# Visual-Behavior/aloception-oss

Measured on AMD Instinct MI355X. Metric: frames/sec (whole node) DeformableDETR-R50 inference, higher is better.
Workload: dtype bf16; 1 GPU; DeformableDETR-R50 inference bf16, batch 8 synthetic 1333x800 frames per GPU, random-init weights; launch=hip-graph replay + eager inference(), per_gpu_batch=8, global_batch=8, parallelism=batch-sharded x1, no collective

## Files before the change

### aloception-oss_amd/alo_hip/__init__.py

```python
import ctypes
import warnings
import os
import subprocess

import torch

_PKG_ROOT = os.path.dirname(os.path.dirname(os.path.abspath(__file__)))
LIB_PATH = os.path.join(_PKG_ROOT, "libalo_hotpath.so")
CSRC_DIR = os.path.join(_PKG_ROOT, "csrc")

ALO_F32, ALO_F64, ALO_BF16, ALO_F16 = 0, 1, 2, 3
RESIDENT_AUTO, RESIDENT_ALWAYS = 0, 1
_DTYPE_CODE = {torch.float32: ALO_F32, torch.float64: ALO_F64, torch.bfloat16: ALO_BF16, torch.float16: ALO_F16}


def _half(f16):
    return (torch.bfloat16, torch.float16) if f16 else (torch.bfloat16,)


_lib = None
_warned_inference_tensor = False


def tensor_version(t):
# ... 685 lines not shown
def linear_shortk_supported(x, weight, f16=False):
    return (x.is_cuda and x.dtype in _half(f16) and weight.dtype == x.dtype and x.shape[-1] in (64, 128, 256)
            and weight.dim() == 2 and weight.shape[1] == x.shape[-1] and weight.shape[0] % 64 == 0)


def linear_shortk(x, weight, bias=None, relu=False, residual=None):
    _no_autograd("linear_shortk", x, weight, bias, residual)
    if not linear_shortk_supported(x, weight, f16=True):
        raise RuntimeError("linear_shortk: needs bf16 / fp16 CUDA tensors of one dtype, K in (64, 128, 256) and N % 64 == 0")
    if bias is not None and bias.dtype != x.dtype:
        raise RuntimeError("linear_shortk: bias must have the dtype of x")
    N, K = weight.shape
    x2 = x.reshape(-1, K)
    if not x2.is_contiguous():
        x2 = x2.contiguous()
    y = torch.empty((x2.shape[0], N), dtype=x.dtype, device=x.device)
    M = x2.shape[0]
    if residual is not None:
        residual = residual.reshape(-1, N)
        if residual.shape[0] != M or residual.dtype != x.dtype or not residual.is_contiguous():
            raise RuntimeError("linear_shortk: residual must be a contiguous (M, N) tensor of x's dtype")
    if M:
        nbytes = 2.0 * (x2.numel() + y.numel() * (2 if residual is not None else 1))
        _launch("alo_linear_shortk", x.device, f"linear_shortk/N={N},K={K}", nbytes, 2.0 * M * N * K, x2, weight.contiguous(),
                None if bias is None else bias.contiguous(), residual, y, M, N, K, 1 if relu else 0, _DTYPE_CODE[x.dtype])
    return y.view(*x.shape[:-1], N)


def linear_packed_supported(x, weight, f16=False):
    return (x.is_cuda and x.dtype in _half(f16) and weight.dtype == x.dtype and weight.dim() == 2
            and x.shape[-1] == weight.shape[1] and weight.shape[1] % 256 == 0 and weight.shape[1] >= 512
            and weight.shape[0] % 128 == 0 and not torch.is_grad_enabled())


def linear_packed(x, weight, bias=None, relu=False, residual=None):
    _no_autograd("linear_packed", x, weight, bias, residual)
    if not linear_packed_supported(x, weight, f16=True):
        raise RuntimeError("linear_packed: needs bf16 / fp16 CUDA tensors of one dtype, K % 256 == 0, K >= 512, N % 128 == 0, no autograd")
    x2 = x.reshape(-1, x.shape[-1])
    if not x2.is_contiguous():
        x2 = x2.contiguous()
    M, K = x2.shape
    N = weight.shape[0]
    y = torch.empty((M, N), dtype=x.dtype, device=x.device)
    if residual is not None:
        residual = residual.reshape(M, N)
        if residual.dtype != x.dtype or not residual.is_contiguous():
            raise RuntimeError("linear_packed: residual must be a contiguous (M, N) tensor of the input's dtype")
    if M:
        packed = pack_mfma_b(weight)
        bias_c = None if bias is None else bias.to(x.dtype).contiguous()
        _launch("alo_linear_packed", x.device, f"linear_packed/K={K}/N={N}", 2.0 * (M * K + M * N * (2 if residual is not None else 1)),
                2.0 * M * N * K, x2, packed, bias_c, residual, y, M, N, K, 1 if relu else 0, _DTYPE_CODE[x.dtype])
    return y.view(*x.shape[:-1], N)


def conv1x1_strided_supported(x, weight2d):
    if not (x.dim() == 4 and x.is_cuda and x.is_contiguous(memory_format=torch.channels_last)):
        return False
    if os.environ.get("ALO_CONV1X1_GATHER") == "0":
        return False
    rows = x.permute(0, 2, 3, 1)
    if linear_shortk_supported(rows, weight2d):
        return True
    return linear_packed_supported(rows, weight2d) and (weight2d.shape[0] >= 1024 or tuple(weight2d.shape) == (128, 512))


def conv1x1_strided(x, weight2d, bias, stride, relu=False):
    _no_autograd("conv1x1_strided", x, weight2d, bias)
    if not conv1x1_strided_supported(x, weight2d):
        raise RuntimeError("conv1x1_strided: unsupported dtype / layout / shape")
    n, cin, h, w_ = x.shape
    cout = weight2d.shape[0]
    ho, wo = (h - 1) // stride + 1, (w_ - 1) // stride + 1
    y = torch.empty((n, cout, ho, wo), dtype=x.dtype, device=x.device, memory_format=torch.channels_last)
    packed = not linear_shortk_supported(x.permute(0, 2, 3, 1), weight2d)
    wt = pack_mfma_b(weight2d) if packed else weight2d.contiguous()
    bias_c = None if bias is None else bias.to(x.dtype).contiguous()
    _launch("alo_conv1x1_nhwc", x.device, f"conv1x1_strided/K={cin}/N={cout}", 2.0 * (y.numel() // cout * cin + y.numel()),
            2.0 * y.numel() * cin, x, wt, 1 if packed else 0, bias_c, None, y, n, h, w_, cin, cout, stride, 1 if relu else 0, ALO_BF16)
    return y


def f32_layers_split():
    return os.environ.get("ALO_F32_LAYERS") == "split"


_F32_ROUTED = {
    (64, 64): (0, None),
    (64, 256): (0, None),
    (256, 128): (0, 1 << 18),
    (256, 256): (0, 1 << 14),
    (256, 384): (0, None),
    (256, 512): (0, None),
    (256, 1024): (1 << 14, None),
    (512, 128): (0, None),
}


def _f32_gemm_routed(M, K, N, identity):
    if identity:
        return K <= 512
    lo, hi = _F32_ROUTED.get((K, N), (0, 0))
    return M >= lo and (hi is None or M < hi)


def linear_f32_supported(x, weight):
    return (x.is_cuda and x.dtype == torch.float32 and weight.dtype == torch.float32 and weight.dim() == 2 and x.dim() >= 1
            and x.shape[-1] == weight.shape[1] and weight.shape[1] % 64 == 0 and weight.shape[0] % 64 == 0 and weight.shape[0] > 0
            and weight.shape[1] > 0 and not needs_autograd(x, weight))


def linear_f32_routed(x, weight, identity=False):
    return (f32_layers_split() and linear_f32_supported(x, weight)
            and _f32_gemm_routed(x.numel() // max(x.shape[-1], 1), weight.shape[1], weight.shape[0], identity))


def _split_weight_of(weight):
    return derived(weight, "linear_f32_b", (weight,), lambda: _split_weight(weight))


def linear_f32(x, weight, bias=None, relu=False, residual=None):
    _no_autograd("linear_f32", x, weight, bias, residual)
    if not linear_f32_supported(x, weight):
        raise RuntimeError("linear_f32: needs fp32 CUDA tensors, a (N, K) weight, K % 64 == 0, N % 64 == 0, no autograd")
    N, K = weight.shape
    x2 = x.reshape(-1, K)
    if not x2.is_contiguous():
        x2 = x2.contiguous()
    M = x2.shape[0]
    y = torch.empty((M, N), dtype=x.dtype, device=x.device)
    if residual is not None:
        residual = residual.reshape(M, N)
        if residual.dtype != x.dtype or not residual.is_contiguous():
            raise RuntimeError("linear_f32: residual must be a contiguous (M, N) fp32 tensor")
    if M:
        bias_c = None if bias is None else bias.float().contiguous()
        _launch("alo_linear_packed", x.device, f"linear_f32/K={K}/N={N}", 4.0 * (M * K + M * N * (2 if residual is not None else 1)),
                2.0 * M * N * K, x2, _split_weight_of(weight), bias_c, residual, y, M, N, K, 1 if relu else 0, ALO_F32)
    return y.view(*x.shape[:-1], N)


def conv1x1_strided_f32(x, weight2d, bias, stride, relu=False):
    _no_autograd("conv1x1_strided_f32", x, weight2d, bias)
    if not (x.dim() == 4 and x.is_contiguous(memory_format=torch.channels_last) and stride >= 1
            and linear_f32_supported(x.permute(0, 2, 3, 1), weight2d)):
        raise RuntimeError("conv1x1_strided_f32: needs a channels-last fp32 CUDA activation, an fp32 (Cout, Cin) weight, Cin % 64 == 0, "
                           "Cout % 64 == 0, no autograd")
    n, cin, h, w_ = x.shape
    cout = weight2d.shape[0]
    ho, wo = (h - 1) // stride + 1, (w_ - 1) // stride + 1
    y = torch.empty((n, cout, ho, wo), dtype=x.dtype, device=x.device, memory_format=torch.channels_last)
    if y.numel():
        bias_c = None if bias is None else bias.float().contiguous()
        _launch("alo_conv1x1_nhwc", x.device, f"conv1x1_strided_f32/K={cin}/N={cout}", 4.0 * (y.numel() // cout * cin + y.numel()),
                2.0 * y.numel() * cin, x, _split_weight_of(weight2d), 1, bias_c, None, y, n, h, w_, cin, cout, stride, 1 if relu else 0, ALO_F32)
    return y


def linear_auto(x, weight, bias=None, relu=False, residual=None):
    _no_autograd("linear_auto", x, weight, bias, residual)
    if linear_shortk_supported(x, weight, f16=True) and (bias is None or bias.dtype == x.dtype):
        return linear_shortk(x, weight, bias, relu, residual=residual)
    if linear_packed_supported(x, weight, f16=True) and (bias is None or bias.dtype == x.dtype) and (
            residual is not None or weight.shape[0] >= 1024 or tuple(weight.shape) == (128, 512)):
        return linear_packed(x, weight, bias, relu, residual=residual)
# ... 519 lines not shown
```

### aloception-oss_amd/alonet/detr/backbone.py

```python
import torch
import torch.nn.functional as F
from torch import nn

import alo_hip

from .misc import assert_and_export_onnx


class FrozenBatchNorm2d(nn.Module):

    def __init__(self, n):
        super().__init__()
        self.register_buffer("weight", torch.ones(n))
        self.register_buffer("bias", torch.zeros(n))
        self.register_buffer("running_mean", torch.zeros(n))
        self.register_buffer("running_var", torch.ones(n))

    def _load_from_state_dict(self, state_dict, prefix, *args, **kwargs):
        state_dict.pop(prefix + "num_batches_tracked", None)
        super()._load_from_state_dict(state_dict, prefix, *args, **kwargs)

    def scale_shift(self):
        scale = self.weight * (self.running_var + 1e-5).rsqrt()
        return scale, self.bias - self.running_mean * scale

    def forward(self, x):
        scale, shift = self.scale_shift()
        return x * scale.reshape(1, -1, 1, 1).to(x.dtype) + shift.reshape(1, -1, 1, 1).to(x.dtype)


def _weight_2d(weight):
    return alo_hip.derived(weight, "2d", (weight,), lambda: weight.reshape(weight.shape[0], -1), no_grad=False)


def conv1x1_as_gemm(x, weight, bias, stride=(1, 1), relu=False, residual=None):
    if tuple(stride) != (1, 1):
        if (stride[0] == stride[1] and residual is None and not torch.is_grad_enabled()
                and alo_hip.conv1x1_strided_supported(x, _weight_2d(weight))):
            return alo_hip.conv1x1_strided(x, _weight_2d(weight), bias, stride[0], relu)
        if (stride[0] == stride[1] and residual is None and alo_hip.f32_layers_split() and x.dim() == 4
                and x.is_contiguous(memory_format=torch.channels_last)
                and alo_hip.linear_f32_supported(x.permute(0, 2, 3, 1), _weight_2d(weight)) and not alo_hip.needs_autograd(bias)):
            return alo_hip.conv1x1_strided_f32(x, _weight_2d(weight), bias, stride[0], relu)
        x = x[:, :, ::stride[0], ::stride[1]]
    n, cin, h, w_ = x.shape
    rows = x.permute(0, 2, 3, 1).reshape(-1, cin)
    res_rows = None if residual is None else residual.permute(0, 2, 3, 1).reshape(-1, weight.shape[0])
    out = alo_hip.linear_auto(rows, _weight_2d(weight), bias, relu, residual=res_rows)
    return out.view(n, h, w_, -1).permute(0, 3, 1, 2)


def folded_conv_bn(conv, bn):
    def fold():
        scale, shift = bn.scale_shift()
        w = (conv.weight.float() * scale.float().reshape(-1, 1, 1, 1)).to(conv.weight.dtype)
        return w.contiguous(memory_format=torch.channels_last), shift.to(conv.weight.dtype)

    if conv.training or torch.is_grad_enabled() and conv.weight.requires_grad:
        return fold()
    return alo_hip.derived(conv, "folded", (conv.weight, bn.weight, bn.bias, bn.running_mean, bn.running_var), fold)


def conv_bn(x, conv, bn, relu=False, residual=None):
    if isinstance(bn, FrozenBatchNorm2d) and conv.bias is None:
        w, b = folded_conv_bn(conv, bn)
        if alo_hip.fusable(x, w, b, residual) and x.is_contiguous(memory_format=torch.channels_last):
            if conv.kernel_size == (1, 1) and conv.padding == (0, 0) and conv.groups == 1 and w.shape[0] % 4 == 0:
                rows_probe = x.permute(0, 2, 3, 1)
                w2 = _weight_2d(w)
                if residual is None or (tuple(conv.stride) == (1, 1) and residual.is_contiguous(memory_format=torch.channels_last)
                                        and (alo_hip.linear_shortk_supported(rows_probe, w2)
                                             or alo_hip.linear_packed_supported(rows_probe, w2)
                                             or alo_hip.linear_f32_routed(rows_probe, w2, identity=True))):
                    return conv1x1_as_gemm(x, w, b, conv.stride, relu=relu, residual=residual)
                out = conv1x1_as_gemm(x, w, None, conv.stride)
                return alo_hip.bias_act_(out, b, residual, relu)
            if residual is None and alo_hip.conv3x3_supported(x, w, conv.stride, conv.padding, conv.dilation, conv.groups):
                return alo_hip.conv3x3(x, w, b, relu, conv.stride)
            if (residual is None and alo_hip.f32_layers_split() and not (conv.stride == (2, 2) and w.shape[1] == 256)
                    and alo_hip.conv3x3_f32_supported(x, w, conv.stride, conv.padding, conv.dilation, conv.groups)):
                return alo_hip.conv3x3_f32(x, w, b, relu, conv.stride)
            if relu or residual is not None:
                out = F.conv2d(x, w, None, conv.stride, conv.padding, conv.dilation, conv.groups)
                if out.is_contiguous(memory_format=torch.channels_last) and out.shape[1] % 4 == 0:
                    return alo_hip.bias_act_(out, b, residual, relu)
                out = out + b.view(1, -1, 1, 1)
            else:
                out = F.conv2d(x, w, b, conv.stride, conv.padding, conv.dilation, conv.groups)
        else:
            out = F.conv2d(x, w, b, conv.stride, conv.padding, conv.dilation, conv.groups)
    else:
        out = bn(conv(x))
    if residual is not None:
        out = out + residual
    return F.relu_(out) if relu else out


class Bottleneck(nn.Module):
    expansion = 4

    def __init__(self, inplanes, planes, stride=1, dilation=1, downsample=None, norm_layer=FrozenBatchNorm2d):
        super().__init__()
        self.conv1 = nn.Conv2d(inplanes, planes, 1, bias=False)
        self.bn1 = norm_layer(planes)
        self.conv2 = nn.Conv2d(planes, planes, 3, stride=stride, padding=dilation, dilation=dilation, bias=False)
        self.bn2 = norm_layer(planes)
        self.conv3 = nn.Conv2d(planes, planes * self.expansion, 1, bias=False)
        self.bn3 = norm_layer(planes * self.expansion)
        self.relu = nn.ReLU(inplace=True)
        self.downsample = downsample

    def forward(self, x):
        identity = x if self.downsample is None else conv_bn(x, self.downsample[0], self.downsample[1])
        out = conv_bn(x, self.conv1, self.bn1, relu=True)
        out = conv_bn(out, self.conv2, self.bn2, relu=True)
        return conv_bn(out, self.conv3, self.bn3, relu=True, residual=identity)


_DEPTHS = {"resnet50": (3, 4, 6, 3), "resnet101": (3, 4, 23, 3)}


class ResNetBody(nn.Module):

    def __init__(self, name="resnet50", replace_stride_with_dilation=(False, False, False),
                 norm_layer=FrozenBatchNorm2d, return_layers=None):
        super().__init__()
        if name not in _DEPTHS:
            raise ValueError(f"backbone {name!r} is not available (have {sorted(_DEPTHS)})")
        self.inplanes, self.dilation = 64, 1
        self.conv1 = nn.Conv2d(3, 64, 7, stride=2, padding=3, bias=False)
        self.bn1 = norm_layer(64)
        self.relu = nn.ReLU(inplace=True)
        self.maxpool = nn.MaxPool2d(3, stride=2, padding=1)
        depths = _DEPTHS[name]
        self.layer1 = self._stage(64, depths[0], 1, False, norm_layer)
        self.layer2 = self._stage(128, depths[1], 2, replace_stride_with_dilation[0], norm_layer)
        self.layer3 = self._stage(256, depths[2], 2, replace_stride_with_dilation[1], norm_layer)
        self.layer4 = self._stage(512, depths[3], 2, replace_stride_with_dilation[2], norm_layer)
        self.return_layers = dict(return_layers or {"layer4": "0"})
        for m in self.modules():
            if isinstance(m, nn.Conv2d):
                nn.init.kaiming_normal_(m.weight, mode="fan_out", nonlinearity="relu")

    def _stage(self, planes, blocks, stride, dilate, norm_layer):
        prev_dilation = self.dilation
        if dilate:
            self.dilation *= stride
            stride = 1
        downsample = None
        if stride != 1 or self.inplanes != planes * Bottleneck.expansion:
            downsample = nn.Sequential(
                nn.Conv2d(self.inplanes, planes * Bottleneck.expansion, 1, stride=stride, bias=False),
                norm_layer(planes * Bottleneck.expansion))
        layers = [Bottleneck(self.inplanes, planes, stride, prev_dilation, downsample, norm_layer)]
        self.inplanes = planes * Bottleneck.expansion
        layers += [Bottleneck(self.inplanes, planes, 1, self.dilation, None, norm_layer) for _ in range(1, blocks)]
        return nn.Sequential(*layers)

    def _stem_fusable(self, x):
        c, p = self.conv1, self.maxpool
        return (alo_hip.stem_conv_pool_supported(x, c.weight) and isinstance(self.bn1, FrozenBatchNorm2d) and c.bias is None
                and c.stride == (2, 2) and c.padding == (3, 3) and c.dilation == (1, 1) and c.groups == 1
                and isinstance(p, nn.MaxPool2d) and p.kernel_size == 3 and p.stride == 2 and p.padding == 1
                and p.dilation == 1 and not p.ceil_mode)

    def forward(self, x):
        out = {}
        if self._stem_fusable(x):
            w, b = folded_conv_bn(self.conv1, self.bn1)
            x = alo_hip.stem_conv_pool(x, w, b)
        else:
            x = x.contiguous(memory_format=torch.channels_last)
            x = self.maxpool(conv_bn(x, self.conv1, self.bn1, relu=True))
        for name in ("layer1", "layer2", "layer3", "layer4"):
            x = getattr(self, name)(x)
            if name in self.return_layers:
                out[self.return_layers[name]] = x
        return out


def _resize_mask(mask, size):
    return F.interpolate(mask, size=size, mode="bilinear", align_corners=False)


class BackboneBase(nn.Module):
    def __init__(self, backbone, train_backbone, num_channels, return_interm_layers, **kwargs):
        super().__init__()
        for name, parameter in backbone.named_parameters():
            if not train_backbone or ("layer2" not in name and "layer3" not in name and "layer4" not in name):
                parameter.requires_grad_(False)
        if return_interm_layers:
            backbone.return_layers = {"layer1": "0", "layer2": "1", "layer3": "2", "layer4": "3"}
        else:
            backbone.return_layers = {"layer4": "0"}
        self.body = backbone
        self.num_channels = num_channels

    def forward(self, frames, skip_masks=False, **kwargs):
        xs = self.body(frames.as_tensor())
        if skip_masks:
            return {name: (x, None) for name, x in xs.items()}
        frame_masks = frames.mask.as_tensor()
        out = {}
        for name, x in xs.items():
            out[name] = (x, _resize_mask(frame_masks.float(), x.shape[-2:]).to(torch.bool))
        return out


class Backbone(BackboneBase):

    def __init__(self, name, train_backbone, return_interm_layers, dilation, **kwargs):
        body = ResNetBody(name, replace_stride_with_dilation=(False, False, dilation), norm_layer=FrozenBatchNorm2d)
        super().__init__(body, train_backbone, 2048, return_interm_layers, **kwargs)


class Joiner(nn.Sequential):

    def __init__(self, backbone, position_embedding, tracing=None):
        super().__init__(backbone, position_embedding)

    @assert_and_export_onnx()
    def forward(self, frames, skip_pos_levels=(), **kwargs):
        out, pos = [], []
        for i, (_, x) in enumerate(self[0](frames, **kwargs).items()):
            out.append(x)
            pos.append(None if i in skip_pos_levels else self[1](x).to(x[0].dtype))
        return out, pos
```

### aloception-oss_amd/csrc/common.hpp

```cpp
#pragma once
#include <hip/hip_runtime.h>
#include <stdint.h>

#include <cstdarg>
#include <cstdio>
#include <type_traits>

#include "../../include/alo_hotpath.h"

namespace alo {

char* error_buffer();
inline int fail(alo_status_t code, const char* fmt, ...) {
    va_list ap;
    va_start(ap, fmt);
    vsnprintf(error_buffer(), 512, fmt, ap);
    va_end(ap);
    return (int)code;
}
#define ALO_REQUIRE(cond, code, ...) \
    do {                             \
        if (!(cond)) return ::alo::fail(code, __VA_ARGS__); \
    } while (0)

template <typename... P>
inline bool aligned16(const P*... p) {
    return ((... | (uintptr_t)p) & 15) == 0;
}

constexpr int kLdsLimit = 160 * 1024;
template <auto kernel>
int launch(dim3 grid, dim3 block, size_t lds, hipStream_t stream, const char* what, void** args) {
    ALO_REQUIRE(lds <= (size_t)kLdsLimit, ALO_ERR_UNSUPPORTED, "%s: %zu bytes of dynamic LDS, the limit is %d", what, lds, kLdsLimit);
    const void* fn = reinterpret_cast<const void*>(kernel);
    hipError_t e = hipSuccess;
    if (lds > 48 * 1024) {
        static unsigned long long done = 0;
        int dev = 0;
        e = hipGetDevice(&dev);
        const unsigned long long bit = 1ull << (dev & 63);
        if (e == hipSuccess && !(__atomic_load_n(&done, __ATOMIC_ACQUIRE) & bit)) {
            e = hipFuncSetAttribute(fn, hipFuncAttributeMaxDynamicSharedMemorySize, kLdsLimit);
            if (e == hipSuccess) __atomic_fetch_or(&done, bit, __ATOMIC_RELEASE);
        }
    }
    if (e == hipSuccess) e = hipLaunchKernel(fn, grid, block, args, lds, stream);
    if (e == hipSuccess) e = hipGetLastError();
    if (e != hipSuccess) return fail(ALO_ERR_LAUNCH, "%s: %s", what, hipGetErrorString(e));
    return ALO_OK;
}

constexpr int kNumXcd = 8;

__device__ __forceinline__ unsigned xcd_contiguous_block(unsigned bid, unsigned nblocks) {
    const unsigned q = nblocks / kNumXcd, r = nblocks % kNumXcd;
    const unsigned xcd = bid % kNumXcd, k = bid / kNumXcd;
    const unsigned start = xcd < r ? xcd * (q + 1) : r * (q + 1) + (xcd - r) * q;
    return start + k;
}

static_assert(kNumXcd == 8, "the tile ranges below shift by 3");
struct TileRange { int first, end, step; };
__device__ __forceinline__ TileRange xcd_tile_range(int ntiles) {
    const int per_xcd = (ntiles + 7) >> 3, xcd = blockIdx.x & 7;
    const int end = (xcd + 1) * per_xcd < ntiles ? (xcd + 1) * per_xcd : ntiles;
    return {(int)(xcd * per_xcd + (blockIdx.x >> 3)), end, (int)(gridDim.x >> 3)};
}
inline unsigned xcd_grid(int ntiles, int max_per_xcd) {
    const int per_xcd = (ntiles + 7) / 8;
    return 8u * (unsigned)(per_xcd < max_per_xcd ? per_xcd : max_per_xcd);
}

struct WidePlan {
    int words[31];
};
bool msda_wide_plan(int N, int S, int M, int D, int Lq, int value_dtype, const int32_t* host_shapes, WidePlan* wp);
int msda_wide_launch(const void* value, const int32_t* shapes, const int32_t* lstart, const void* loc, const void* attn,
                     const void* grad_out, void* grad_value, void* grad_loc, void* grad_attn, const WidePlan& wp, int D,
                     int value_dtype, hipStream_t stream);

struct RowGather {
    int s, Wo, HoWo, W, HW;
};
inline RowGather row_gather(int stride = 1, int Ho = 1, int Wo = 1, int H = 1, int W = 1) { return {stride, Wo, Ho * Wo, W, H * W}; }

int linear_shortk_gather(const void* x, const void* weight, const void* bias, const void* residual, void* y, long M, int N, int K,
                         int relu, const RowGather& gather, hipStream_t stream);

int conv3x3_f32(const void* x, const void* w_split, const void* bias, void* y, void* image_mag, int N, int H, int W, int Cin, int Cout,
                int stride, int relu, hipStream_t stream);

int linear_f32(const void* x, const void* w_split, const void* bias, const void* residual, void* y, long M, int N, int K, int relu,
               const RowGather& gather, hipStream_t stream, const char* what);

int ffn_f32(const void* x, const void* w1_split, const void* b1, const void* w2_split, const void* b2, void* y, long M, int F,
            hipStream_t stream, const char* what);

#define ALO_RELU_RES(fn, first, relu, residual, ...)                                                                          \
    ((residual) ? ((relu) ? fn<first, true, true>(__VA_ARGS__) : fn<first, false, true>(__VA_ARGS__))                          \
                : ((relu) ? fn<first, true, false>(__VA_ARGS__) : fn<first, false, false>(__VA_ARGS__)))

typedef __attribute__((ext_vector_type(4))) unsigned int u32x4;
typedef __attribute__((ext_vector_type(2))) unsigned int u32x2;
typedef __attribute__((ext_vector_type(4))) float f32x4;
typedef __attribute__((ext_vector_type(16))) float f32x16;

struct bf16_t {
    uint16_t bits;
};

__device__ __forceinline__ float relu_keep_nan(float v) { return (v > 0.f || v != v) ? v : 0.f; }

__device__ __forceinline__ float bf16_to_f32(uint16_t b) { return __uint_as_float(((unsigned)b) << 16); }
__device__ __forceinline__ uint16_t f32_to_bf16(float f) {
    const __bf16 b = static_cast<__bf16>(f);
    return __builtin_bit_cast(uint16_t, b);
}
__device__ __forceinline__ unsigned pack_bf16x2(float lo, float hi) {
    typedef __bf16 bf16x2_hw __attribute__((ext_vector_type(2)));
    typedef float f32x2_hw __attribute__((ext_vector_type(2)));
    const bf16x2_hw r = __builtin_convertvector(f32x2_hw{lo, hi}, bf16x2_hw);
    return __builtin_bit_cast(unsigned, r);
}

struct f16_t {
    uint16_t bits;
};
__device__ __forceinline__ float f16_to_f32(uint16_t b) { return (float)__builtin_bit_cast(_Float16, b); }
__device__ __forceinline__ uint16_t f32_to_f16(float f) {
    const _Float16 h = static_cast<_Float16>(f);
    return __builtin_bit_cast(uint16_t, h);
}
__device__ __forceinline__ unsigned pack_f16x2(float lo, float hi) {
    typedef _Float16 f16x2_hw __attribute__((ext_vector_type(2)));
    typedef float f32x2_hw __attribute__((ext_vector_type(2)));
    const f16x2_hw r = __builtin_convertvector(f32x2_hw{lo, hi}, f16x2_hw);
    return __builtin_bit_cast(unsigned, r);
}
template <typename T>
__device__ __forceinline__ void unpack2(unsigned w, float& lo, float& hi) {
    if constexpr (std::is_same<T, f16_t>::value) {
        lo = f16_to_f32((uint16_t)(w & 0xffffu));
        hi = f16_to_f32((uint16_t)(w >> 16));
    } else {
        lo = __uint_as_float(w << 16);
        hi = __uint_as_float(w & 0xffff0000u);
    }
}
template <typename T>
__device__ __forceinline__ unsigned pack2(float lo, float hi) {
    if constexpr (std::is_same<T, f16_t>::value) return pack_f16x2(lo, hi);
    else return pack_bf16x2(lo, hi);
}
template <typename T>
__device__ __forceinline__ void unpack4(const u32x2& x, float (&v)[4]) {
    unpack2<T>(x.x, v[0], v[1]);
    unpack2<T>(x.y, v[2], v[3]);
}
template <typename T>
__device__ __forceinline__ u32x2 pack4(const float (&v)[4]) { return u32x2{pack2<T>(v[0], v[1]), pack2<T>(v[2], v[3])}; }

template <typename F>
inline int with_storage_type(int dtype, F&& f) {
    return dtype == ALO_F16 ? f(f16_t{}) : f(bf16_t{});
}

typedef __attribute__((ext_vector_type(8))) __bf16 bf16x8_t;
__device__ __forceinline__ bf16x8_t as_bf16x8(const u32x4& v) {
    union { u32x4 u; bf16x8_t b; } x;
    x.u = v;
    return x.b;
// ... 168 lines not shown
```

### aloception-oss_amd/csrc/gemm_packed.hip

```cpp
#include "mfma_tile.hpp"

namespace alo {
namespace {

constexpr int kOutStride = 64 * 2 + 16;

template <typename T, int kWC>
struct Packed {
    using type = T;
    static constexpr int WC = kWC;
};

struct PackedDims {
    long M;
    int N, K;
    RowGather g;
};

template <typename T, int WC, bool RELU, bool HAS_RES>
__global__ void __launch_bounds__(256, 2)
linear_packed_kernel(const T* __restrict__ X, const T* __restrict__ Wp, const T* __restrict__ bias, const T* __restrict__ R,
                     T* __restrict__ Y, const PackedDims dm) {
    constexpr int WR = 4 / WC;
    constexpr int kRows = 64 * WR;
// ... 50 lines not shown

    const int nchunks = dm.K / KC;
    const int total_batches = nchunks * NB;
    u32x4 stage[kLoads];
    u32x4 bufa[2][KB], bufb[2][KB];
    fetch(0, stage);
    load_batch(bufa, wfrag, tile_stride, 0);
    for (int c = 0; c < nchunks; ++c) {
        park_tile<kPieces>(xs, kStride, stage, tid);
        __syncthreads();
        if (c + 1 < nchunks) fetch(c + 1, stage);
        const int gb = c * NB;
#pragma unroll
        for (int bt = 0; bt < NB; bt += 2) {
            load_batch(bufb, wfrag, tile_stride, gb + bt + 1);
            mma_batch(bufa, bt);
            if (gb + bt + 2 < total_batches) load_batch(bufa, wfrag, tile_stride, gb + bt + 2);
            mma_batch(bufb, bt + 1);
        }
        __syncthreads();
    }

    stage_quads<T, true>(obuf, kOutStride, acc, bias_s + wc * 64, RELU && !HAS_RES, nl, 0, kg);
    wave_lds_fence();
    store_rows<T, RELU, HAS_RES>(Y, R, obuf, kOutStride, row0 + 64 * wr, dm.M, dm.N, col0, lane);
}

template <class Cfg, bool RELU, bool HAS_RES>
int launch_packed(const void* x, const void* w, const void* bias, const void* residual, void* y, const PackedDims& dm, hipStream_t stream) {
    constexpr int WC = Cfg::WC, WR = 4 / WC, kRows = 64 * WR, KC = 256 / WR;
    constexpr size_t xbytes = (size_t)kRows * (KC * 2 + 16), obytes = 4 * 64 * kOutStride;
    constexpr size_t lds = (xbytes > obytes ? xbytes : obytes) + 256 * sizeof(float);
    void* args[] = {&x, &w, &bias, &residual, &y, const_cast<PackedDims*>(&dm)};
    const dim3 grid((unsigned)((dm.M + kRows - 1) / kRows), (unsigned)(dm.N / (64 * WC)));
    return launch<linear_packed_kernel<typename Cfg::type, WC, RELU, HAS_RES>>(grid, 256, lds, stream, "alo_linear_packed", args);
}

template <typename T>
int dispatch_packed(const void* x, const void* w_packed, const void* bias, const void* residual, void* y, const PackedDims& dm,
                    int relu, void* stream) {
    hipStream_t s = static_cast<hipStream_t>(stream);
    using Wide = Packed<T, 4>;
    using Square = Packed<T, 2>;
    if (dm.N % 256 == 0) return ALO_RELU_RES(launch_packed, Wide, relu, residual, x, w_packed, bias, residual, y, dm, s);
    return ALO_RELU_RES(launch_packed, Square, relu, residual, x, w_packed, bias, residual, y, dm, s);
}

}
}

using namespace alo;

extern "C" int alo_linear_packed(const void* x, const void* w_packed, const void* bias, const void* residual, void* y, long M,
                                 int N, int K, int relu, int dtype, void* stream) {
    ALO_REQUIRE(dtype == ALO_BF16 || dtype == ALO_F16 || dtype == ALO_F32, ALO_ERR_UNSUPPORTED,
                "alo_linear_packed: bf16 / fp16, or fp32 with split weights, only (dtype %d)", dtype);
    ALO_REQUIRE(x && w_packed && y, ALO_ERR_INVALID_ARGUMENT, "alo_linear_packed: null pointer argument");
    ALO_REQUIRE(M > 0 && N > 0 && K > 0, ALO_ERR_INVALID_ARGUMENT, "alo_linear_packed: sizes must be positive");
    if (dtype == ALO_F32) {
        ALO_REQUIRE(K % 64 == 0 && N % 64 == 0, ALO_ERR_UNSUPPORTED, "alo_linear_packed: fp32 needs K and N to be multiples of 64 (K=%d N=%d)", K, N);
        ALO_REQUIRE(aligned16(x, w_packed, y, residual), ALO_ERR_INVALID_ARGUMENT, "alo_linear_packed: pointers must be 16-byte aligned");
        ALO_REQUIRE((M + 63) / 64 < (1L << 28), ALO_ERR_UNSUPPORTED, "alo_linear_packed: too many rows");
        return linear_f32(x, w_packed, bias, residual, y, M, N, K, relu, row_gather(), static_cast<hipStream_t>(stream), "alo_linear_packed");
    }
    ALO_REQUIRE(K % 256 == 0 && N % 128 == 0, ALO_ERR_UNSUPPORTED,
                "alo_linear_packed: K must be a multiple of 256 and N of 128 (K=%d N=%d)", K, N);
    ALO_REQUIRE(aligned16(x, w_packed, y, residual), ALO_ERR_INVALID_ARGUMENT, "alo_linear_packed: pointers must be 16-byte aligned");
    ALO_REQUIRE((M + 63) / 64 < (1L << 31), ALO_ERR_UNSUPPORTED, "alo_linear_packed: too many rows");
    PackedDims dm;
    dm.M = M; dm.N = N; dm.K = K; dm.g = row_gather();
    return with_storage_type(dtype, [&](auto t) { return dispatch_packed<decltype(t)>(x, w_packed, bias, residual, y, dm, relu, stream); });
}

extern "C" int alo_conv1x1_nhwc(const void* x, const void* weight, int weight_is_packed, const void* bias, const void* residual,
                                void* y, int N, int H, int W, int Cin, int Cout, int stride, int relu, int dtype, void* stream) {
    ALO_REQUIRE(x && weight && y, ALO_ERR_INVALID_ARGUMENT, "alo_conv1x1_nhwc: null pointer argument");
    ALO_REQUIRE(N > 0 && H > 0 && W > 0 && stride >= 1, ALO_ERR_INVALID_ARGUMENT, "alo_conv1x1_nhwc: N, H, W, stride must be positive");
    ALO_REQUIRE(dtype == ALO_BF16 || dtype == ALO_F32, ALO_ERR_UNSUPPORTED,
                "alo_conv1x1_nhwc: bf16 only, or fp32 with split packed weights (dtype %d)", dtype);
    ALO_REQUIRE(aligned16(x, weight, y, residual), ALO_ERR_INVALID_ARGUMENT, "alo_conv1x1_nhwc: pointers must be 16-byte aligned");
    const int Ho = (H - 1) / stride + 1, Wo = (W - 1) / stride + 1;
    const long M = (long)N * Ho * Wo;
    ALO_REQUIRE((long)H * W < (1L << 30), ALO_ERR_UNSUPPORTED, "alo_conv1x1_nhwc: map too large");
    const RowGather gather = row_gather(stride, Ho, Wo, H, W);
    if (dtype == ALO_F32) {
        ALO_REQUIRE(weight_is_packed, ALO_ERR_UNSUPPORTED, "alo_conv1x1_nhwc: fp32 takes the split packed weight only (weight_is_packed = 1)");
        ALO_REQUIRE(Cin > 0 && Cout > 0 && Cin % 64 == 0 && Cout % 64 == 0, ALO_ERR_UNSUPPORTED,
                    "alo_conv1x1_nhwc: fp32 needs Cin and Cout to be multiples of 64 (Cin=%d Cout=%d)", Cin, Cout);
        ALO_REQUIRE((M + 63) / 64 < (1L << 28), ALO_ERR_UNSUPPORTED, "alo_conv1x1_nhwc: too many output pixels");
        return linear_f32(x, weight, bias, residual, y, M, Cout, Cin, relu, gather, static_cast<hipStream_t>(stream), "alo_conv1x1_nhwc");
    }
    if (!weight_is_packed) {
        ALO_REQUIRE(Cout % 64 == 0, ALO_ERR_UNSUPPORTED, "alo_conv1x1_nhwc: Cout must be a multiple of 64 (got %d)", Cout);
        return linear_shortk_gather(x, weight, bias, residual, y, M, Cout, Cin, relu, gather, static_cast<hipStream_t>(stream));
    }
    ALO_REQUIRE(Cin % 256 == 0 && Cout % 128 == 0, ALO_ERR_UNSUPPORTED,
                "alo_conv1x1_nhwc: packed weights need Cin %% 256 == 0 and Cout %% 128 == 0 (Cin=%d Cout=%d)", Cin, Cout);
    PackedDims dm;
    dm.M = M; dm.N = Cout; dm.K = Cin; dm.g = gather;
    return dispatch_packed<bf16_t>(x, weight, bias, residual, y, dm, relu, stream);
}
```

### include/alo_hotpath.h

```cpp
#ifndef ALO_HOTPATH_H
#define ALO_HOTPATH_H

#include <stddef.h>
#include <stdint.h>

#ifdef __cplusplus
extern "C" {
#endif

#define ALO_HOTPATH_ABI_VERSION 3

typedef enum alo_status {
    ALO_OK = 0,
    ALO_ERR_INVALID_ARGUMENT = 1,
    ALO_ERR_UNSUPPORTED = 2,
    ALO_ERR_LAUNCH = 3
} alo_status_t;

typedef enum alo_dtype {
    ALO_F32 = 0,
    ALO_F64 = 1,
    ALO_BF16 = 2,
    ALO_F16 = 3
} alo_dtype_t;
// ... 5 lines not shown
int alo_msda_forward(const void* value, const int32_t* spatial_shapes, const int32_t* level_start_index,
                     const void* sampling_loc, const void* attn_weight, void* out,
                     int N, int S, int M, int D, int L, int Lq, int P,
                     int value_dtype, int loc_dtype, void* stream);

int alo_msda_forward_fused(const void* value, const int32_t* spatial_shapes, const int32_t* level_start_index,
                           const void* sampling_offsets, const void* attn_logits, const void* reference_points,
                           void* out, int N, int S, int M, int D, int L, int Lq, int P, int ref_dim,
                           int value_dtype, void* stream);

int alo_msda_forward_fused_hm(const void* value_hm, const int32_t* spatial_shapes, const int32_t* level_start_index,
                              const void* sampling_offsets, const void* attn_logits, const void* reference_points,
                              void* out, int N, int S, int M, int D, int L, int Lq, int P, int ref_dim,
                              int value_dtype, void* stream);
int alo_msda_forward_fused_hm_rows(const void* value_hm, const int32_t* spatial_shapes, const int32_t* level_start_index,
                                   const void* sampling_offsets, const void* attn_logits, long offsets_row_elems,
                                   long logits_row_elems, const void* reference_points, void* out, int N, int S, int M, int D,
                                   int L, int Lq, int P, int ref_dim, int value_dtype, void* stream);

#define ALO_RESIDENT_AUTO 0
#define ALO_RESIDENT_ALWAYS 1
int alo_msda_forward_fused_hm_resident(const void* value_hm, const int32_t* spatial_shapes, const int32_t* level_start_index,
                                       const void* sampling_offsets, const void* attn_logits, long offsets_row_elems,
                                       long logits_row_elems, const void* reference_points, void* out, int N, int S, int M, int D,
                                       int L, int Lq, int P, int ref_dim, int value_dtype, const int32_t* host_spatial_shapes,
                                       int policy, void* stream);
int alo_msda_resident_levels(const int32_t* host_spatial_shapes, int N, int S, int M, int L, int Lq, int policy);

int alo_value_head_major(const void* value, const void* padding_mask, void* out, int N, int S, int M, int D,
                         int dtype, void* stream);

int alo_msda_backward(const void* value, const int32_t* spatial_shapes, const int32_t* level_start_index,
                      const void* sampling_loc, const void* attn_weight, const void* grad_out,
                      void* grad_value, void* grad_sampling_loc, void* grad_attn_weight,
                      int N, int S, int M, int D, int L, int Lq, int P,
                      int value_dtype, int loc_dtype, void* stream);

int alo_msda_backward_hinted(const void* value, const int32_t* spatial_shapes, const int32_t* level_start_index,
                             const void* sampling_loc, const void* attn_weight, const void* grad_out,
                             void* grad_value, void* grad_sampling_loc, void* grad_attn_weight,
                             int N, int S, int M, int D, int L, int Lq, int P,
                             int value_dtype, int loc_dtype, const int32_t* host_spatial_shapes, void* stream);

#define ALO_MSDA_BWD_GENERIC 0
#define ALO_MSDA_BWD_TILED 1
#define ALO_MSDA_BWD_WIDE 2
int alo_msda_backward_path(int N, int S, int M, int D, int L, int Lq, int P, int value_dtype, int loc_dtype,
                           const int32_t* host_spatial_shapes);

void alo_corr_level_shape(int H, int W, int level, int* h_out, int* w_out);

size_t alo_corr_build_workspace_bytes(int B, int C, int H, int W, int num_levels);

int alo_corr_build(const float* fmap1, const float* fmap2, float* const* levels, void* workspace,
                   size_t workspace_bytes, int B, int C, int H, int W, int num_levels, void* stream);

int alo_corr_lookup(const float* const* levels, const float* coords, float* out,
                    int B, int H, int W, int radius, int num_levels, void* stream);

int alo_corr_lookup_backward(float* const* grad_levels, const float* coords, const float* grad_out,
                             int B, int H, int W, int radius, int num_levels, void* stream);

int alo_corr_lookup_backward_coords(const float* const* levels, const float* coords, const float* grad_out,
                                    float* grad_coords_levels, int B, int H, int W, int radius, int num_levels, void* stream);

int alo_add_layernorm(const void* x, const void* residual, const void* gamma, const void* beta, void* out,
                      const void* pos, void* out_pos, long rows, int C, float eps, int dtype, void* stream);
int alo_bias_act(const void* x, const void* bias, const void* residual, void* y, long rows, int C, int relu,
                 int dtype, void* stream);

int alo_linear_shortk(const void* x, const void* weight, const void* bias, const void* residual, void* y, long M, int N,
                      int K, int relu, int dtype, void* stream);

int alo_value_proj_head_major(const void* x, const void* weight, const void* bias, const void* padding_mask, void* value_hm,
                              int batch, int S, int heads, int K, int dtype, void* stream);

int alo_pack_mfma_b(const void* w, void* packed, int N, int K, int dtype, void* stream);
int alo_ffn256(const void* x, const void* w1, const void* b1, const void* w2, const void* b2, void* y, long M, int F,
               int dtype, void* stream);

int alo_linear_packed(const void* x, const void* w_packed, const void* bias, const void* residual, void* y, long M, int N, int K,
                      int relu, int dtype, void* stream);

int alo_conv1x1_nhwc(const void* x, const void* weight, int weight_is_packed, const void* bias, const void* residual, void* y, int N,
                     int H, int W, int Cin, int Cout, int stride, int relu, int dtype, void* stream);

int alo_conv3x3_small_nhwc(const void* x, const void* w_frag, const void* bias32, void* y, int N, int H, int W, int Cin, int Cout,
                           int dtype, void* stream);

size_t alo_conv3x3_workspace_bytes(int N, int H, int W, int Cin, int Cout, int stride);
int alo_conv3x3_nhwc(const void* x, const void* w_packed, const void* bias, void* y, void* workspace, int N, int H, int W, int Cin,
                     int Cout, int stride, int relu, int dtype, void* stream);

int alo_stem_conv_pool(const void* x, const void* w_packed, const void* bias, void* y, int N, int H, int W, long stride_n,
                       long stride_c, long stride_h, long stride_w, int dtype, void* stream);

size_t alo_groupnorm_rows_workspace_bytes(int B, int HW, int groups);
int alo_groupnorm_rows(const void* x, const void* weight, const void* bias, void* y, void* workspace, int B, int HW, int C,
                       int groups, float eps, long y_batch_stride, int dtype, void* stream);
int alo_groupnorm_rows_act(const void* x, const void* weight, const void* bias, void* y, void* workspace, int B, int HW, int C,
                           int groups, float eps, long y_batch_stride, int relu, int dtype, void* stream);

int alo_upsample_add_nhwc(const void* x_low, const void* fpn, void* out, int BQ, int Q, int C, int h, int w, int H, int W, int dtype,
                          void* stream);

int alo_mask_pyramid(const void* frame_mask, int mask_is_float, unsigned char* mask_flat, float* valid_ratios, int B, int H, int W,
                     int L, const int* level_shapes_host, unsigned nearest_levels, void* stream);
int alo_encoder_reference_points(const float* valid_ratios, float* reference_points, int B, int L, const int* level_shapes_host,
                                 void* stream);

int alo_panoptic_onehot(const float* mask_logits, long long* onehot, int B, int Q, int h, int w, int H, int W, float threshold,
                        void* stream);

int alo_pos_sine_flat(const void* padding_mask, const int32_t* spatial_shapes, const int32_t* level_start_index,
                      const float* dim_t, const void* level_embed, void* out, float* workspace, int B, int S, int L,
                      int num_pos_feats, int normalize, int center, float scale, float eps, int dtype, void* stream);

int alo_bias_act_nchw(const float* x, const float* bias, float* y, int B, int C, int HW, int relu, void* stream);
int alo_gru_gate(float* zr, const float* bias_zr, const float* h, float* rh, int B, int C, int HW,
                 long h_batch_stride, long rh_batch_stride, void* stream);
int alo_gru_update(const float* q, const float* bias_q, const float* zr, float* h, float* net, int B, int C, int HW,
                   long h_batch_stride, void* stream);

#ifdef __cplusplus
}
#endif
#endif
```

Before: 928.4 frames/s.

## Fuse bottleneck conv3, downsample/residual and next block's conv1 into one kernel

Adds a fused HIP kernel for ResNet layer1-style bottlenecks (64->256 1x1). It computes conv3 with the residual add or the downsample conv, then the next block's 256->64/128 conv1 from the tile already held in LDS. The backbone loop now threads that precomputed head into the next block. This removes separate launches and an HBM round trip of the 256-channel output feeding the next conv1. The cost is a specialized kernel, heavier LDS and register use, and more complex block dispatch.

New measurement: 953.2 frames/s (median of 6 runs). 1.03x the previous value.

```diff
diff --git a/aloception-oss_amd/alo_hip/__init__.py b/aloception-oss_amd/alo_hip/__init__.py
--- a/aloception-oss_amd/alo_hip/__init__.py
+++ b/aloception-oss_amd/alo_hip/__init__.py
@@ -791,6 +791,60 @@
     return y
 
 
+CONV1X1_CHAIN, CONV1X1_CHAIN_DOWN = 2, 4
+
+
+def bottleneck_chain_enabled():
+    return os.environ.get("ALO_BOTTLENECK_CHAIN", "on").lower() not in ("off", "0")
+
+
+def _chain_map(t, channels):
+    return (t.dim() == 4 and t.is_cuda and t.dtype == torch.bfloat16 and t.shape[1] == channels and t.numel() > 0
+            and t.is_contiguous(memory_format=torch.channels_last))
+
+
+def _chain_vectors(*pairs):
+    return all(w.dtype == torch.bfloat16 and tuple(w.shape[:2]) == (cout, cin) and w.numel() == cout * cin
+               and b is not None and b.dtype == torch.bfloat16 and tuple(b.shape) == (cout,) for w, b, cout, cin in pairs)
+
+
+def conv1x1_chain_supported(mid, conv3, identity=None, down=None, nxt=None):
+    if (identity is None) == (down is None) or not bottleneck_chain_enabled() or torch.is_grad_enabled():
+        return False
+    other = identity if down is None else down[0]
+    if not (_chain_map(mid, 64) and _chain_map(other, 256 if down is None else 64) and other.shape[0] == mid.shape[0]
+            and other.shape[2:] == mid.shape[2:] and other.device == mid.device):
+        return False
+    pairs = [(*conv3, 256, 64)] + ([] if down is None else [(down[1], down[2], 256, 64)])
+    if nxt is not None:
+        if nxt[0].shape[0] not in (64, 128):
+            return False
+        pairs.append((*nxt, nxt[0].shape[0], 256))
+    return _chain_vectors(*pairs) and fusable(mid, other, *[t for w, b, _, _ in pairs for t in (w, b)])
+
+
+def conv1x1_chain(mid, conv3, identity=None, down=None, nxt=None):
+    _no_autograd("conv1x1_chain", mid, *conv3, identity, *(down or ()), *(nxt or ()))
+    if not conv1x1_chain_supported(mid, conv3, identity, down, nxt):
+        raise RuntimeError("conv1x1_chain: needs channels-last bf16 CUDA maps outside autograd, a 64 -> 256 convolution, an identity or "
+                           "a 64 -> 256 downsample convolution, a next convolution 256 -> 64 or 128, and ALO_BOTTLENECK_CHAIN not off")
+    n, _, h, w_ = mid.shape
+    n2 = 0 if nxt is None else nxt[0].shape[0]
+    parts = [*conv3, *(down[1:] if down is not None else ()), *(nxt or ())]
+    buf = derived(conv3[0], f"chain/{down is not None}/{n2}", parts, lambda: torch.cat([p.reshape(-1) for p in parts]))
+    rows = n * h * w_
+    out = torch.empty(rows * (256 + n2), dtype=mid.dtype, device=mid.device)
+    other = identity if down is None else down[0]
+    nbytes = 2.0 * rows * (64 + (256 if down is None else 64) + 256 + n2)
+    flops = 2.0 * rows * 256 * (64 * (1 + (down is not None)) + n2)
+    tag = f"conv1x1_chain/{'down' if down is not None else 'res'}{f'+next{n2}' if n2 else ''}"
+    _launch("alo_conv1x1_nhwc", mid.device, tag, nbytes, flops, mid, buf, CONV1X1_CHAIN | (CONV1X1_CHAIN_DOWN if down is not None else 0) | n2,
+            None, other, out, n, h, w_, 64, 256, 1, 1, ALO_BF16)
+    y = out[:rows * 256].view(n, h, w_, 256).permute(0, 3, 1, 2)
+    z = None if nxt is None else out[rows * 256:].view(n, h, w_, n2).permute(0, 3, 1, 2)
+    return y, z
+
+
 def f32_layers_split():
     return os.environ.get("ALO_F32_LAYERS") == "split"
 
diff --git a/aloception-oss_amd/alonet/detr/backbone.py b/aloception-oss_amd/alonet/detr/backbone.py
--- a/aloception-oss_amd/alonet/detr/backbone.py
+++ b/aloception-oss_amd/alonet/detr/backbone.py
@@ -96,6 +96,9 @@
     return F.relu_(out) if relu else out
 
 
+_conv_bn = conv_bn
+
+
 class Bottleneck(nn.Module):
     expansion = 4
 
@@ -110,11 +113,41 @@
         self.relu = nn.ReLU(inplace=True)
         self.downsample = downsample
 
-    def forward(self, x):
-        identity = x if self.downsample is None else conv_bn(x, self.downsample[0], self.downsample[1])
-        out = conv_bn(x, self.conv1, self.bn1, relu=True)
+    def _chain(self, x, mid, nxt):
+        def pointwise(conv, bn):
+            return (isinstance(bn, FrozenBatchNorm2d) and conv.bias is None and conv.kernel_size == (1, 1) and conv.stride == (1, 1)
+                    and conv.padding == (0, 0) and conv.groups == 1)
+
+        if not (conv_bn is _conv_bn and alo_hip.bottleneck_chain_enabled() and not torch.is_grad_enabled()
+                and x.is_cuda and x.dtype == torch.bfloat16 and pointwise(self.conv3, self.bn3)
+                and alo_hip.fusable(x, mid, self.conv3, self.bn3, self.downsample)):
+            return None
+        down = identity = head = None
+        if self.downsample is None:
+            identity = x
+        elif len(self.downsample) == 2 and pointwise(self.downsample[0], self.downsample[1]):
+            down = (x, *folded_conv_bn(self.downsample[0], self.downsample[1]))
+        else:
+            return None
+        if isinstance(nxt, Bottleneck) and pointwise(nxt.conv1, nxt.bn1) and alo_hip.fusable(x, nxt.conv1, nxt.bn1):
+            head = folded_conv_bn(nxt.conv1, nxt.bn1)
+            if head[0].shape[0] not in (64, 128):
+                head = None
+        if down is None and head is None:
+            return None
+        args = (mid, folded_conv_bn(self.conv3, self.bn3), identity, down, head)
+        return args if alo_hip.conv1x1_chain_supported(*args) else None
+
+    def forward(self, x, head=None, nxt=None):
+        out = conv_bn(x, self.conv1, self.bn1, relu=True) if head is None else head
         out = conv_bn(out, self.conv2, self.bn2, relu=True)
-        return conv_bn(out, self.conv3, self.bn3, relu=True, residual=identity)
+        chain = self._chain(x, out, nxt)
+        if chain is not None:
+            out, head = alo_hip.conv1x1_chain(*chain)
+        else:
+            identity = x if self.downsample is None else conv_bn(x, self.downsample[0], self.downsample[1])
+            out, head = conv_bn(out, self.conv3, self.bn3, relu=True, residual=identity), None
+        return out if nxt is None else (out, head)
 
 
 _DEPTHS = {"resnet50": (3, 4, 6, 3), "resnet101": (3, 4, 23, 3)}
@@ -173,7 +206,13 @@
             x = x.contiguous(memory_format=torch.channels_last)
             x = self.maxpool(conv_bn(x, self.conv1, self.bn1, relu=True))
         for name in ("layer1", "layer2", "layer3", "layer4"):
-            x = getattr(self, name)(x)
+            stage = getattr(self, name)
+            head = None
+            for i, block in enumerate(stage):
+                if i + 1 < len(stage):
+                    x, head = block(x, head=head, nxt=stage[i + 1])
+                else:
+                    x = block(x, head=head)
             if name in self.return_layers:
                 out[self.return_layers[name]] = x
         return out
diff --git a/aloception-oss_amd/csrc/common.hpp b/aloception-oss_amd/csrc/common.hpp
--- a/aloception-oss_amd/csrc/common.hpp
+++ b/aloception-oss_amd/csrc/common.hpp
@@ -87,6 +87,8 @@
 int linear_shortk_gather(const void* x, const void* weight, const void* bias, const void* residual, void* y, long M, int N, int K,
                          int relu, const RowGather& gather, hipStream_t stream);
 
+int conv1x1_chain(const void* mid, const void* w_chain, const void* res_or_x0, void* y, long M, bool down, int n2, hipStream_t stream);
+
 int conv3x3_f32(const void* x, const void* w_split, const void* bias, void* y, void* image_mag, int N, int H, int W, int Cin, int Cout,
                 int stride, int relu, hipStream_t stream);
 
diff --git a/aloception-oss_amd/csrc/conv1x1_chain.hip b/aloception-oss_amd/csrc/conv1x1_chain.hip
--- /dev/null
+++ b/aloception-oss_amd/csrc/conv1x1_chain.hip
@@ -0,0 +1,249 @@
+#include "mfma_tile.hpp"
+
+namespace alo {
+namespace {
+
+constexpr int kRows = 64;
+constexpr int kK = 64;
+constexpr int kN = 256;
+constexpr int kInStride = kK * 2 + 16;
+constexpr int kOutStride = 64 * 2 + 16;
+constexpr int kSteps = kK / 16;
+constexpr int kPieces = kK / 8;
+constexpr int kLoads = kRows * kPieces / 256;
+constexpr int kNextSteps = kN / 16;
+
+struct ChainArgs {
+    const bf16_t *X, *X0, *R;
+    const bf16_t *W3, *B3, *Wd, *Bd, *W1, *B1;
+    bf16_t *Y, *Z;
+    long M;
+    int tiles;
+};
+
+constexpr int z_stride(int n2) { return n2 * 2 + 16; }
+constexpr size_t chain_lds(bool down, int n2) {
+    return (size_t)kRows * kInStride * (down ? 2 : 1) + 4 * kRows * kOutStride + (n2 ? kRows * z_stride(n2) : 0) +
+           (4 * 64 * (down ? 2 : 1) + (n2 ? 4 * 32 : 0)) * sizeof(float);
+}
+
+template <bool DOWN, int N2>
+__global__ void __launch_bounds__(256, 2) conv1x1_chain_kernel(const ChainArgs a) {
+    using T = bf16_t;
+    static_assert(N2 == 0 || N2 == 64 || N2 == 128, "the next convolution has 64 or 128 output channels");
+    static_assert(kRows * kPieces % 256 == 0, "the tile loader gives every thread the same number of pieces");
+    constexpr int kZStride = z_stride(N2);
+    extern __shared__ __attribute__((aligned(16))) unsigned char smem[];
+    const int tid = threadIdx.x, wave = tid >> 6, lane = tid & 63;
+    const int nl = lane & 31, kg = lane >> 5;
+    unsigned char* const xbuf = smem;
+    unsigned char* const x0buf = smem + kRows * kInStride;
+    unsigned char* const ytile = x0buf + (DOWN ? kRows * kInStride : 0);
+    unsigned char* const obuf = ytile + wave * (kRows * kOutStride);
+    unsigned char* const zbuf = ytile + 4 * kRows * kOutStride;
+    float* const tabs = reinterpret_cast<float*>(zbuf + (N2 ? kRows * kZStride : 0));
+    float* const b3_tab = tabs + wave * 64;
+    float* const bd_tab = tabs + 4 * 64 + wave * 64;
+    float* const b1_tab = tabs + 4 * 64 * (DOWN ? 2 : 1) + wave * 32;
+    const int col0 = wave * 64;
+
+    u32x4 w3[2][kSteps];
+    [[maybe_unused]] u32x4 wd[DOWN ? 2 : 1][kSteps];
+#pragma unroll
+    for (int t = 0; t < 2; ++t)
+#pragma unroll
+        for (int s = 0; s < kSteps; ++s) {
+            w3[t][s] = *reinterpret_cast<const u32x4*>(a.W3 + (size_t)(col0 + 32 * t + nl) * kK + 8 * kg + 16 * s);
+            if constexpr (DOWN) wd[t][s] = *reinterpret_cast<const u32x4*>(a.Wd + (size_t)(col0 + 32 * t + nl) * kK + 8 * kg + 16 * s);
+        }
+    {
+        const int r = lane & 15, t = (lane >> 4) & 1, k2 = lane >> 5;
+        const int c = col0 + 32 * t + (r & 3) + 8 * (r >> 2) + 4 * k2;
+        b3_tab[lane] = ld(&a.B3[c]);
+        if constexpr (DOWN) bd_tab[lane] = ld(&a.Bd[c]);
+    }
+    constexpr int kHalves = N2 == 128 ? 2 : 1;
+    const int zcol0 = N2 == 128 ? 32 * wave : 32 * (wave & 1);
+    const int zhalf0 = N2 == 128 ? 0 : wave >> 1;
+    [[maybe_unused]] u32x4 w1[N2 ? kNextSteps : 1];
+    if constexpr (N2 != 0) {
+#pragma unroll
+        for (int s = 0; s < kNextSteps; ++s)
+            w1[s] = *reinterpret_cast<const u32x4*>(a.W1 + (size_t)(zcol0 + nl) * kN + 8 * kg + 16 * s);
+        if (lane < 32) {
+            const int r = lane & 15, k2 = lane >> 4;
+            b1_tab[lane] = ld(&a.B1[zcol0 + (r & 3) + 8 * (r >> 2) + 4 * k2]);
+        }
+    }
+
+    auto fetch = [&](const T* X, int tile, u32x4 (&r)[kLoads]) {
+#pragma unroll
+        for (int j = 0; j < kLoads; ++j) {
+            const int p = tid + 256 * j;
+            long row = (long)tile * kRows + p / kPieces;
+            row = row < a.M ? row : a.M - 1;
+            r[j] = *reinterpret_cast<const u32x4*>(X + row * kK + (p % kPieces) * 8);
+        }
+    };
+
+    int tile = blockIdx.x;
+    if (tile >= a.tiles) return;
+    u32x4 stage[kLoads];
+    [[maybe_unused]] u32x4 stage0[DOWN ? kLoads : 1];
+    fetch(a.X, tile, stage);
+    if constexpr (DOWN) fetch(a.X0, tile, stage0);
+
+    for (;;) {
+        park_tile<kPieces>(xbuf, kInStride, stage, tid);
+        if constexpr (DOWN) park_tile<kPieces>(x0buf, kInStride, stage0, tid);
+        __syncthreads();
+        const long grow0 = (long)tile * kRows;
+        const int next = tile + gridDim.x;
+        const bool more = next < a.tiles;
+        [[maybe_unused]] u32x4 idn[DOWN ? 1 : 8];
+        if constexpr (!DOWN) fetch_identity(idn, a.R, grow0, a.M, kN, col0, lane);
+        if (more) {
+            fetch(a.X, next, stage);
+            if constexpr (DOWN) fetch(a.X0, next, stage0);
+        }
+
+#pragma unroll
+        for (int half = 0; half < kRows / 32; ++half) {
+            f32x16 acc[2];
+            [[maybe_unused]] f32x16 accd[DOWN ? 2 : 1];
+#pragma unroll
+            for (int t = 0; t < 2; ++t)
+#pragma unroll
+                for (int q = 0; q < 4; ++q) {
+                    const f32x4 b4 = *reinterpret_cast<const f32x4*>(b3_tab + (kg * 2 + t) * 16 + 4 * q);
+#pragma unroll
+                    for (int i = 0; i < 4; ++i) acc[t][4 * q + i] = b4[i];
+                    if constexpr (DOWN) {
+                        const f32x4 d4 = *reinterpret_cast<const f32x4*>(bd_tab + (kg * 2 + t) * 16 + 4 * q);
+#pragma unroll
+                        for (int i = 0; i < 4; ++i) accd[t][4 * q + i] = d4[i];
+                    }
+                }
+#pragma unroll
+            for (int s = 0; s < kSteps; ++s) {
+                const int off = (32 * half + nl) * kInStride + (16 * s + 8 * kg) * 2;
+                const u32x4 f = *reinterpret_cast<const u32x4*>(xbuf + off);
+                acc[0] = mfma_32x32x16<T>(w3[0][s], f, acc[0]);
+                acc[1] = mfma_32x32x16<T>(w3[1][s], f, acc[1]);
+                if constexpr (DOWN) {
+                    const u32x4 f0 = *reinterpret_cast<const u32x4*>(x0buf + off);
+                    accd[0] = mfma_32x32x16<T>(wd[0][s], f0, accd[0]);
+                    accd[1] = mfma_32x32x16<T>(wd[1][s], f0, accd[1]);
+                }
+            }
+            if constexpr (DOWN) {
+#pragma unroll
+                for (int t = 0; t < 2; ++t)
+#pragma unroll
+                    for (int q = 0; q < 4; ++q) {
+                        unsigned o[2];
+#pragma unroll
+                        for (int i = 0; i < 2; ++i) {
+                            float plo, phi, dlo, dhi;
+                            unpack2<T>(pack2<T>(acc[t][4 * q + 2 * i], acc[t][4 * q + 2 * i + 1]), plo, phi);
+                            unpack2<T>(pack2<T>(accd[t][4 * q + 2 * i], accd[t][4 * q + 2 * i + 1]), dlo, dhi);
+                            o[i] = pack2<T>(relu_keep_nan(plo + dlo), relu_keep_nan(phi + dhi));
+                        }
+                        *reinterpret_cast<u32x2*>(obuf + (32 * half + nl) * kOutStride + (32 * t + 8 * q + 4 * kg) * 2) = u32x2{o[0], o[1]};
+                    }
+            } else {
+                stage_quads<T, false>(obuf, kOutStride, acc, nullptr, false, 32 * half + nl, 0, kg);
+            }
+        }
+        wave_lds_fence();
+#pragma unroll
+        for (int pass = 0; pass < 8; ++pass) {
+            const int row = pass * 8 + (lane >> 3);
+            unsigned char* const at = obuf + row * kOutStride + (lane & 7) * 16;
+            u32x4 v = *reinterpret_cast<const u32x4*>(at);
+            if constexpr (!DOWN) {
+                v = add_residual_x8<T, true>(v, idn[pass]);
+                if constexpr (N2 != 0) *reinterpret_cast<u32x4*>(at) = v;
+            }
+            if (grow0 + row < a.M) *reinterpret_cast<u32x4*>(a.Y + (grow0 + row) * kN + col0 + (lane & 7) * 8) = v;
+        }
+
+        if constexpr (N2 != 0) {
+            __syncthreads();
+            f32x16 accz[kHalves];
+#pragma unroll
+            for (int h = 0; h < kHalves; ++h)
+#pragma unroll
+                for (int q = 0; q < 4; ++q) {
+                    const f32x4 b4 = *reinterpret_cast<const f32x4*>(b1_tab + kg * 16 + 4 * q);
+#pragma unroll
+                    for (int i = 0; i < 4; ++i) accz[h][4 * q + i] = b4[i];
+                }
+#pragma unroll
+            for (int s = 0; s < kNextSteps; ++s) {
+                const unsigned char* const blk = ytile + (s >> 2) * (kRows * kOutStride) + (16 * (s & 3) + 8 * kg) * 2;
+#pragma unroll
+                for (int h = 0; h < kHalves; ++h) {
+                    const u32x4 f = *reinterpret_cast<const u32x4*>(blk + (32 * (zhalf0 + h) + nl) * kOutStride);
+                    accz[h] = mfma_32x32x16<T>(w1[s], f, accz[h]);
+                }
+            }
+#pragma unroll
+            for (int h = 0; h < kHalves; ++h)
+#pragma unroll
+                for (int q = 0; q < 4; ++q) {
+                    const float v0 = relu_keep_nan(accz[h][4 * q]), v1 = relu_keep_nan(accz[h][4 * q + 1]);
+                    const float v2 = relu_keep_nan(accz[h][4 * q + 2]), v3 = relu_keep_nan(accz[h][4 * q + 3]);
+                    *reinterpret_cast<u32x2*>(zbuf + (32 * (zhalf0 + h) + nl) * kZStride + (zcol0 + 8 * q + 4 * kg) * 2) =
+                        u32x2{pack2<T>(v0, v1), pack2<T>(v2, v3)};
+                }
+            __syncthreads();
+            constexpr int kZPieces = N2 / 8;
+#pragma unroll
+            for (int j = 0; j < kRows * kZPieces / 256; ++j) {
+                const int p = tid + 256 * j, row = p / kZPieces, piece = p % kZPieces;
+                if (grow0 + row < a.M)
+                    *reinterpret_cast<u32x4*>(a.Z + (grow0 + row) * N2 + piece * 8) =
+                        *reinterpret_cast<const u32x4*>(zbuf + row * kZStride + piece * 16);
+            }
+            if (!more) break;
+        } else {
+            if (!more) break;
+            __syncthreads();
+        }
+        tile = next;
+    }
+}
+
+template <bool DOWN, int N2>
+int launch_chain(const ChainArgs& a, hipStream_t stream) {
+    int gx = a.tiles < 512 ? a.tiles : 512;
+    void* args[] = {const_cast<ChainArgs*>(&a)};
+    return launch<conv1x1_chain_kernel<DOWN, N2>>(gx, 256, chain_lds(DOWN, N2), stream, "alo_conv1x1_nhwc", args);
+}
+
+}
+}
+
+int alo::conv1x1_chain(const void* mid, const void* w_chain, const void* res_or_x0, void* y, long M, bool down, int n2, hipStream_t stream) {
+    const bf16_t* w = static_cast<const bf16_t*>(w_chain);
+    ChainArgs a{};
+    a.X = static_cast<const bf16_t*>(mid);
+    (down ? a.X0 : a.R) = static_cast<const bf16_t*>(res_or_x0);
+    a.W3 = w; w += kN * kK;
+    a.B3 = w; w += kN;
+    if (down) {
+        a.Wd = w; w += kN * kK;
+        a.Bd = w; w += kN;
+    }
+    if (n2) {
+        a.W1 = w; w += (size_t)n2 * kN;
+        a.B1 = w;
+    }
+    a.Y = static_cast<bf16_t*>(y);
+    a.Z = n2 ? a.Y + M * kN : nullptr;
+    a.M = M;
+    a.tiles = (int)((M + kRows - 1) / kRows);
+    if (down) return n2 == 128 ? launch_chain<true, 128>(a, stream) : n2 == 64 ? launch_chain<true, 64>(a, stream) : launch_chain<true, 0>(a, stream);
+    return n2 == 128 ? launch_chain<false, 128>(a, stream) : n2 == 64 ? launch_chain<false, 64>(a, stream) : launch_chain<false, 0>(a, stream);
+}
diff --git a/aloception-oss_amd/csrc/gemm_packed.hip b/aloception-oss_amd/csrc/gemm_packed.hip
--- a/aloception-oss_amd/csrc/gemm_packed.hip
+++ b/aloception-oss_amd/csrc/gemm_packed.hip
@@ -156,6 +156,25 @@
     const int Ho = (H - 1) / stride + 1, Wo = (W - 1) / stride + 1;
     const long M = (long)N * Ho * Wo;
     ALO_REQUIRE((long)H * W < (1L << 30), ALO_ERR_UNSUPPORTED, "alo_conv1x1_nhwc: map too large");
+    if (weight_is_packed & ALO_CONV1X1_CHAIN) {
+        const bool down = (weight_is_packed & ALO_CONV1X1_CHAIN_DOWN) != 0;
+        const int n2 = weight_is_packed & ~(ALO_CONV1X1_CHAIN | ALO_CONV1X1_CHAIN_DOWN);
+        ALO_REQUIRE(dtype == ALO_BF16 && Cin == 64 && Cout == 256 && stride == 1 && relu && (n2 == 0 || n2 == 64 || n2 == 128),
+                    ALO_ERR_UNSUPPORTED,
+                    "alo_conv1x1_nhwc: a chain buffer needs bf16, Cin = 64, Cout = 256, stride 1, relu and a next width of 0, 64 or 128 "
+                    "(dtype %d Cin=%d Cout=%d stride=%d relu=%d next=%d)", dtype, Cin, Cout, stride, relu, n2);
+        ALO_REQUIRE(residual && !bias, ALO_ERR_INVALID_ARGUMENT,
+                    "alo_conv1x1_nhwc: a chain buffer carries its biases (bias must be NULL) and needs the identity, or the downsample "
+                    "convolution's input, in residual");
+        ALO_REQUIRE((M + 63) / 64 < (1L << 31), ALO_ERR_UNSUPPORTED, "alo_conv1x1_nhwc: too many output pixels");
+        const size_t rows = (size_t)M;
+        const struct { const void* p; size_t bytes; } out = {y, rows * 2 * (256 + (size_t)n2)},
+                                                      ins[] = {{x, rows * 128}, {residual, rows * (down ? 128 : 512)}};
+        for (const auto& i : ins)
+            ALO_REQUIRE((const char*)out.p + out.bytes <= (const char*)i.p || (const char*)i.p + i.bytes <= (const char*)out.p,
+                        ALO_ERR_INVALID_ARGUMENT, "alo_conv1x1_nhwc: the output of a chain overlaps an input");
+        return conv1x1_chain(x, weight, residual, y, M, down, n2, static_cast<hipStream_t>(stream));
+    }
     const RowGather gather = row_gather(stride, Ho, Wo, H, W);
     if (dtype == ALO_F32) {
         ALO_REQUIRE(weight_is_packed, ALO_ERR_UNSUPPORTED, "alo_conv1x1_nhwc: fp32 takes the split packed weight only (weight_is_packed = 1)");
diff --git a/include/alo_hotpath.h b/include/alo_hotpath.h
--- a/include/alo_hotpath.h
+++ b/include/alo_hotpath.h
@@ -111,6 +111,8 @@
 int alo_linear_packed(const void* x, const void* w_packed, const void* bias, const void* residual, void* y, long M, int N, int K,
                       int relu, int dtype, void* stream);
 
+#define ALO_CONV1X1_CHAIN 2
+#define ALO_CONV1X1_CHAIN_DOWN 4
 int alo_conv1x1_nhwc(const void* x, const void* weight, int weight_is_packed, const void* bias, const void* residual, void* y, int N,
                      int H, int W, int Cin, int Cout, int stride, int relu, int dtype, void* stream);
 
```
